# MengLcool/RichSem

Measured on AMD Instinct MI355X. Metric: training images/sec, RichSem R50 4-scale 1333x800 (MSDeformAttn hot path: 12 fwd + 12 bwd calls per step), higher is better.
Workload: dtype f32; 1 GPU; configs[1]: R50 4-scale 800x1344 (S=22323), bs=2/GPU, M=8 D=32 L=P=4; per step 6x E(Lq=22323) + 6x Dd(Lq=1092), forward and backward, 12 distinct per-layer tensor sets; loc-init; loc=init, images_per_gpu=2, parallelism=dp1 (replicas, no collective)

## Files before the change

richsem_amd/csrc/msda_direct.h:

```cpp
#pragma once

#include "msda_common.h"
#include "msda_prep.h"

namespace msda {

struct DirectGeom {
    int N, S, M, D, L, Lq, P;
    int G, logG, nchunks;
    int qtile, ntiles;
    int pbatch;
    unsigned gv_skip;
};

constexpr int kDirectThreads = 256;
constexpr int kDirectWaves = kDirectThreads / kWave;
constexpr int kMinGroup = 8;

template <typename T>
inline size_t direct_lds_bytes(const DirectGeom &g)
{
    const int ipw = kWave / g.G;
    return sizeof(LevelGeom) * g.L + sizeof(PointRec<T>) * kDirectWaves * ipw * (g.pbatch + 1);
}

__device__ __forceinline__ void load_levels(LevelGeom *lv, const int64_t *shapes, const int64_t *lsi, int L)
{
    for (int l = threadIdx.x; l < L; l += blockDim.x) {
        lv[l].H = (int)shapes[2 * l];
        lv[l].W = (int)shapes[2 * l + 1];
        lv[l].start = (int)lsi[l];
        lv[l].pad = 0;
    }
    __syncthreads();
}

template <typename T, int C, int OCC, typename TV = T>
__global__ __launch_bounds__(kDirectThreads, OCC) void fwd_direct_kernel(
    const TV *__restrict__ value, const int64_t *__restrict__ shapes, const int64_t *__restrict__ lsi,
    const T *__restrict__ loc, const T *__restrict__ aw, TV *__restrict__ out, const DirectGeom g)
{
    extern __shared__ __attribute__((aligned(16))) unsigned char smem[];
    LevelGeom *lv = reinterpret_cast<LevelGeom *>(smem);
    PointRec<T> *recs = reinterpret_cast<PointRec<T> *>(smem + sizeof(LevelGeom) * g.L);

    int pair, tile;
    if (!decode_block(blockIdx.x, g.N * g.M, g.ntiles, pair, tile)) return;
    load_levels(lv, shapes, lsi, g.L);

    const int b = pair / g.M, m = pair - b * g.M;
    const int lane = threadIdx.x & (kWave - 1), wave = threadIdx.x / kWave;
    const int ipw = kWave >> g.logG;
    const int j = lane & (g.G - 1);
    const int slot = wave * ipw + (lane >> g.logG);
    const int LP = g.L * g.P;
    const int row_elems = g.M * g.D;
    PointRec<T> *my = recs + slot * (g.pbatch + 1);

    const int q_end = min((tile + 1) * g.qtile, g.Lq);
    for (int q0 = tile * g.qtile; q0 < q_end; q0 += kDirectWaves * ipw) {
        const int q = q0 + slot;
        const bool live = q < q_end;
        const int item = (b * g.Lq + q) * g.M + m;
        for (int ch = 0; ch < g.nchunks; ++ch) {
            const int c0 = (ch * g.G + j) * C;
            const bool has_c = live && c0 < g.D;
            T acc[C];
#pragma unroll
            for (int c = 0; c < C; ++c) acc[c] = (T)0;
            for (int p0 = 0; p0 < LP; p0 += g.pbatch) {
                const int np = min(g.pbatch, LP - p0);
                if (live) {
                    for (int pt = j; pt < np; pt += g.G) {
                        const int gp = p0 + pt, l = gp / g.P;
                        const Pack<T, 2> xy = *reinterpret_cast<const Pack<T, 2> *>(loc + ((int64_t)item * LP + gp) * 2);
                        const T a = aw[(int64_t)item * LP + gp];
                        const LevelGeom G_ = lv[l];
                        PointRec<T> r;
                        T lh, lw;
                        resolve_point<T>(xy.v[0], xy.v[1], G_.H, G_.W,
                                         (b * g.S + G_.start) * row_elems + m * g.D,
                                         row_elems, r.o, lh, lw);
                        const T hh = (T)1 - lh, hw = (T)1 - lw;
                        r.f[0] = hh * hw * a;
                        r.f[1] = hh * lw * a;
                        r.f[2] = lh * hw * a;
                        r.f[3] = lh * lw * a;
                        my[pt] = r;
                    }
                }
                __builtin_amdgcn_wave_barrier();
                if (has_c) {
#pragma unroll(OCC >= 6 ? 2 : 4)
                    for (int pt = 0; pt < np; ++pt) {
                        const PointRec<T> r = my[pt];
                        Pack<T, C> v[4];
#pragma unroll
                        for (int k = 0; k < 4; ++k) {
                            if (r.o[k] >= 0) {
                                const Pack<TV, C> raw = *reinterpret_cast<const Pack<TV, C> *>(value + r.o[k] + c0);
#pragma unroll
                                for (int c = 0; c < C; ++c) v[k].v[c] = to_compute<T, TV>(raw.v[c]);
                            } else {
#pragma unroll
                                for (int c = 0; c < C; ++c) v[k].v[c] = (T)0;
                            }
                        }
#pragma unroll
                        for (int c = 0; c < C; ++c)
                            acc[c] += r.f[0] * v[0].v[c] + r.f[1] * v[1].v[c] + r.f[2] * v[2].v[c] + r.f[3] * v[3].v[c];
                    }
                }
                __builtin_amdgcn_wave_barrier();
            }
            if (has_c) {
                Pack<TV, C> o;
#pragma unroll
                for (int c = 0; c < C; ++c) o.v[c] = to_storage<TV, T>(acc[c]);
                *reinterpret_cast<Pack<TV, C> *>(out + (int64_t)item * g.D + c0) = o;
            }
        }
    }
}

constexpr int kSplitGroups = 4;
constexpr int kSplitMaxPts = 8;
template <typename TV, int PPG>
__global__ __launch_bounds__(kDirectThreads, 4) void fwd_split_kernel(
    const TV *__restrict__ value, const int64_t *__restrict__ shapes, const int64_t *__restrict__ lsi,
    const float *__restrict__ loc, const float *__restrict__ aw, TV *__restrict__ out, const DirectGeom g)
{
    extern __shared__ __attribute__((aligned(16))) unsigned char smem[];
    LevelGeom *lv = reinterpret_cast<LevelGeom *>(smem);
    load_levels(lv, shapes, lsi, g.L);
    const int lane = threadIdx.x & (kWave - 1);
    const int j = lane & 7, pg = (lane >> 3) & (kSplitGroups - 1);
    const long long n_items = (long long)g.N * g.Lq * g.M;
    const long long item_raw = ((long long)blockIdx.x * kDirectThreads + threadIdx.x) >> 5;
    const bool live = item_raw < n_items;
    const long long item = live ? item_raw : n_items - 1;
    const int m = (int)(item % g.M);
    const int b = (int)(item / ((long long)g.Lq * g.M));
    const int LP = g.L * g.P, ppg = PPG ? PPG : LP / kSplitGroups;
    const int row_elems = g.M * g.D, c0 = 4 * j;
    float acc[4] = {0.f, 0.f, 0.f, 0.f};
#pragma unroll
    for (int i = 0; i < (PPG ? PPG : kSplitMaxPts); ++i) {
        if (!PPG && i >= ppg) break;
        const int gp = pg * ppg + i, l = gp / g.P;
        const Pack<float, 2> xy = *reinterpret_cast<const Pack<float, 2> *>(loc + (item * LP + gp) * 2);
        const float a = aw[item * LP + gp];
        const LevelGeom G_ = lv[l];
        int o[4];
        float lh, lw;
        resolve_point<float>(xy.v[0], xy.v[1], G_.H, G_.W, (b * g.S + G_.start) * row_elems + m * g.D, row_elems, o, lh, lw);
        const float hh = 1.f - lh, hw = 1.f - lw;
        const float f[4] = {hh * hw * a, hh * lw * a, lh * hw * a, lh * lw * a};
#pragma unroll
        for (int k = 0; k < 4; ++k) {
            const Pack<TV, 4> raw = *reinterpret_cast<const Pack<TV, 4> *>(value + (o[k] >= 0 ? o[k] : (b * g.S) * row_elems + m * g.D) + c0);
#pragma unroll
            for (int c = 0; c < 4; ++c) acc[c] += f[k] * (o[k] >= 0 ? to_compute<float, TV>(raw.v[c]) : 0.f);
        }
    }
#pragma unroll
    for (int c = 0; c < 4; ++c) {
        acc[c] += dpp_f<0x128>(acc[c]);
        acc[c] += __shfl_xor(acc[c], 16, kWave);
    }
    if (live && pg == 0) {
        Pack<TV, 4> o_;
#pragma unroll
        for (int c = 0; c < 4; ++c) o_.v[c] = to_storage<TV, float>(acc[c]);
        *reinterpret_cast<Pack<TV, 4> *>(out + item * g.D + c0) = o_;
    }
}

template <typename TP>
struct PrepSrc {
    const TP *offsets, *logits;
    long long off_stride, log_stride;
    int ref_dim;
};

template <typename T, int C, int OCC, typename TV, typename TP>
__global__ __launch_bounds__(kDirectThreads, OCC) void fwd_direct_prep_kernel(
    const TV *__restrict__ value, const int64_t *__restrict__ shapes, const int64_t *__restrict__ lsi, const PrepSrc<TP> src,
    const T *__restrict__ ref, T *__restrict__ loc_out, T *__restrict__ aw_out, TV *__restrict__ out, const DirectGeom g)
{
    extern __shared__ __attribute__((aligned(16))) unsigned char smem[];
    LevelGeom *lv = reinterpret_cast<LevelGeom *>(smem);
    PointRec<T> *recs = reinterpret_cast<PointRec<T> *>(smem + sizeof(LevelGeom) * g.L);

    int pair, tile;
    if (!decode_block(blockIdx.x, g.N * g.M, g.ntiles, pair, tile)) return;
    load_levels(lv, shapes, lsi, g.L);

    const int b = pair / g.M, m = pair - b * g.M;
    const int lane = threadIdx.x & (kWave - 1), wave = threadIdx.x / kWave;
    const int ipw = kWave >> g.logG;
    const int j = lane & (g.G - 1);
    const int slot = wave * ipw + (lane >> g.logG);
    const int LP = g.L * g.P;
    const int row_elems = g.M * g.D;
    PointRec<T> *my = recs + slot * (g.pbatch + 1);
    constexpr int kPerLane = kPointBatch / kMinGroup;

    const int q_end = min((tile + 1) * g.qtile, g.Lq);
    for (int q0 = tile * g.qtile; q0 < q_end; q0 += kDirectWaves * ipw) {
        const int q = q0 + slot;
        const bool live = q < q_end;
        const long long nq = (long long)b * g.Lq + (live ? q : q_end - 1);
        const long long item = nq * g.M + m;
        T lg[kPerLane];
        T mx = (T)-3.0e38;
#pragma unroll
        for (int i = 0; i < kPerLane; ++i) {
            const int pt = j + i * g.G;
            lg[i] = pt < LP ? prep_ld<T>(src.logits + nq * src.log_stride + (long long)m * LP + pt) : (T)-3.0e38;
            mx = lg[i] > mx ? lg[i] : mx;
        }
        for (int s_ = 1; s_ < g.G; s_ <<= 1) {
            const T o = __shfl_xor(mx, s_, kWave);
            mx = o > mx ? o : mx;
        }
        T sum = (T)0;
#pragma unroll
        for (int i = 0; i < kPerLane; ++i) {
            lg[i] = j + i * g.G < LP ? exp(lg[i] - mx) : (T)0;
            sum += lg[i];
        }
        for (int s_ = 1; s_ < g.G; s_ <<= 1) sum += __shfl_xor(sum, s_, kWave);
#pragma unroll
        for (int i = 0; i < kPerLane; ++i) {
            const int pt = j + i * g.G;
            if (live && pt < LP) {
                const int l = pt / g.P;
                const T a = lg[i] / sum;
                const TP *o = src.offsets + nq * src.off_stride + ((long long)m * LP + pt) * 2;
                const T ox = prep_ld<T>(o), oy = prep_ld<T>(o + 1);
                const T *r = ref + (nq * g.L + l) * src.ref_dim;
                const LevelGeom G_ = lv[l];
                T lx, ly;
                if (src.ref_dim == 2) {
                    lx = r[0] + ox / (T)G_.W;
                    ly = r[1] + oy / (T)G_.H;
                } else {
                    lx = r[0] + ox / (T)g.P * r[2] * (T)0.5;
                    ly = r[1] + oy / (T)g.P * r[3] * (T)0.5;
                }
                if (loc_out) {
                    Pack<T, 2> xy;
                    xy.v[0] = lx;
                    xy.v[1] = ly;
                    *reinterpret_cast<Pack<T, 2> *>(loc_out + (item * LP + pt) * 2) = xy;
                    aw_out[item * LP + pt] = a;
                }
                PointRec<T> rec;
                T lh, lw;
                resolve_point<T>(lx, ly, G_.H, G_.W, (b * g.S + G_.start) * row_elems + m * g.D, row_elems, rec.o, lh, lw);
                const T hh = (T)1 - lh, hw = (T)1 - lw;
                rec.f[0] = hh * hw * a;
                rec.f[1] = hh * lw * a;
                rec.f[2] = lh * hw * a;
                rec.f[3] = lh * lw * a;
                my[pt] = rec;
            }
        }
        __builtin_amdgcn_wave_barrier();
        for (int ch = 0; ch < g.nchunks; ++ch) {
            const int c0 = (ch * g.G + j) * C;
            if (live && c0 < g.D) {
                T acc[C];
#pragma unroll
                for (int c = 0; c < C; ++c) acc[c] = (T)0;
#pragma unroll(OCC >= 6 ? 2 : 4)
                for (int pt = 0; pt < LP; ++pt) {
                    const PointRec<T> r = my[pt];
                    Pack<T, C> v[4];
#pragma unroll
                    for (int k = 0; k < 4; ++k) {
                        if (r.o[k] >= 0) {
                            const Pack<TV, C> raw = *reinterpret_cast<const Pack<TV, C> *>(value + r.o[k] + c0);
#pragma unroll
                            for (int c = 0; c < C; ++c) v[k].v[c] = to_compute<T, TV>(raw.v[c]);
                        } else {
#pragma unroll
                            for (int c = 0; c < C; ++c) v[k].v[c] = (T)0;
                        }
                    }
#pragma unroll
                    for (int c = 0; c < C; ++c)
                        acc[c] += r.f[0] * v[0].v[c] + r.f[1] * v[1].v[c] + r.f[2] * v[2].v[c] + r.f[3] * v[3].v[c];
                }
                Pack<TV, C> o;
#pragma unroll
                for (int c = 0; c < C; ++c) o.v[c] = to_storage<TV, T>(acc[c]);
                *reinterpret_cast<Pack<TV, C> *>(out + item * g.D + c0) = o;
            }
        }
        __builtin_amdgcn_wave_barrier();
    }
}

template <typename TV, int PPG, int THREADS>
__device__ __forceinline__ void bwd_split_body(unsigned bid, const LevelGeom *lv, const TV *__restrict__ value,
                                               const float *__restrict__ loc, const float *__restrict__ aw, const TV *__restrict__ grad_out,
                                               float *__restrict__ grad_loc, float *__restrict__ grad_aw, const DirectGeom &g)
{
    const int lane = threadIdx.x & (kWave - 1);
    const int j = lane & 7, pg = (lane >> 3) & (kSplitGroups - 1);
    const long long n_items = (long long)g.N * g.Lq * g.M;
    const long long item_raw = ((long long)bid * THREADS + threadIdx.x) >> 5;
    const bool live = item_raw < n_items;
    const long long item = live ? item_raw : n_items - 1;
    const int m = (int)(item % g.M);
    const int b = (int)(item / ((long long)g.Lq * g.M));
    const int LP = g.L * g.P, ppg = PPG ? PPG : LP / kSplitGroups;
    const int row_elems = g.M * g.D, c0 = 4 * j;
    float go[4];
    {
        const Pack<TV, 4> raw = *reinterpret_cast<const Pack<TV, 4> *>(grad_out + item * g.D + c0);
#pragma unroll
        for (int c = 0; c < 4; ++c) go[c] = to_compute<float, TV>(raw.v[c]);
    }
    float r_a[PPG ? PPG : kSplitMaxPts], r_w[PPG ? PPG : kSplitMaxPts], r_h[PPG ? PPG : kSplitMaxPts];
#pragma unroll
    for (int i = 0; i < (PPG ? PPG : kSplitMaxPts); ++i) {
        if (!PPG && i >= ppg) break;
        const int gp = pg * ppg + i, l = gp / g.P;
        const Pack<float, 2> xy = *reinterpret_cast<const Pack<float, 2> *>(loc + (item * LP + gp) * 2);
        const float a = aw[item * LP + gp];
        const LevelGeom G_ = lv[l];
        int o[4];
        float lh, lw;
        resolve_point<float>(xy.v[0], xy.v[1], G_.H, G_.W, (b * g.S + G_.start) * row_elems + m * g.D, row_elems, o, lh, lw);
        const float hh = 1.f - lh, hw = 1.f - lw;
        float v[4][4];
#pragma unroll
        for (int k = 0; k < 4; ++k) {
            const Pack<TV, 4> raw = *reinterpret_cast<const Pack<TV, 4> *>(value + (o[k] >= 0 ? o[k] : (b * g.S) * row_elems + m * g.D) + c0);
#pragma unroll
            for (int c = 0; c < 4; ++c) v[k][c] = o[k] >= 0 ? to_compute<float, TV>(raw.v[c]) : 0.f;
        }
        float s_a = 0.f, s_w = 0.f, s_h = 0.f;
#pragma unroll
        for (int c = 0; c < 4; ++c) {
            const float tgv = go[c] * a;
            s_a += go[c] * (hh * hw * v[0][c] + hh * lw * v[1][c] + lh * hw * v[2][c] + lh * lw * v[3][c]);
            s_w += (hh * (v[1][c] - v[0][c]) + lh * (v[3][c] - v[2][c])) * tgv;
            s_h += (hw * (v[2][c] - v[0][c]) + lw * (v[3][c] - v[1][c])) * tgv;
        }
        r_a[i] = group8_sum(s_a);
        r_w[i] = (float)G_.W * group8_sum(s_w);
        r_h[i] = (float)G_.H * group8_sum(s_h);
        if (!PPG && live && j == 0) {
            grad_aw[item * LP + gp] = r_a[i];
            Pack<float, 2> gl;
            gl.v[0] = r_w[i];
            gl.v[1] = r_h[i];
            *reinterpret_cast<Pack<float, 2> *>(grad_loc + (item * LP + gp) * 2) = gl;
        }
    }
    if (PPG && live && j == 0) {
#pragma unroll
        for (int i = 0; i < PPG; ++i) {
            const int gp = pg * PPG + i;
            grad_aw[item * LP + gp] = r_a[i];
            Pack<float, 2> gl;
            gl.v[0] = r_w[i];
            gl.v[1] = r_h[i];
            *reinterpret_cast<Pack<float, 2> *>(grad_loc + (item * LP + gp) * 2) = gl;
        }
    }
}

template <typename TV, int PPG>
__global__ __launch_bounds__(kDirectThreads, 4) void bwd_split_kernel(
    const TV *__restrict__ value, const int64_t *__restrict__ shapes, const int64_t *__restrict__ lsi,
    const float *__restrict__ loc, const float *__restrict__ aw, const TV *__restrict__ grad_out,
    float *__restrict__ grad_loc, float *__restrict__ grad_aw, const DirectGeom g)
{
    extern __shared__ __attribute__((aligned(16))) unsigned char smem[];
    LevelGeom *lv = reinterpret_cast<LevelGeom *>(smem);
    load_levels(lv, shapes, lsi, g.L);
    bwd_split_body<TV, PPG, kDirectThreads>(blockIdx.x, lv, value, loc, aw, grad_out, grad_loc, grad_aw, g);
}

template <typename T, int C, typename TV = T>
__global__ __launch_bounds__(kDirectThreads) void bwd_direct_kernel(
    const TV *__restrict__ value, const int64_t *__restrict__ shapes, const int64_t *__restrict__ lsi,
    const T *__restrict__ loc, const T *__restrict__ aw, const TV *__restrict__ grad_out,
    T *__restrict__ grad_value, T *__restrict__ grad_loc, T *__restrict__ grad_aw, const DirectGeom g)
{
    extern __shared__ __attribute__((aligned(16))) unsigned char smem[];
    LevelGeom *lv = reinterpret_cast<LevelGeom *>(smem);
    PointRec<T> *recs = reinterpret_cast<PointRec<T> *>(smem + sizeof(LevelGeom) * g.L);

    int pair, tile;
    if (!decode_block(blockIdx.x, g.N * g.M, g.ntiles, pair, tile)) return;
    load_levels(lv, shapes, lsi, g.L);

    const int b = pair / g.M, m = pair - b * g.M;
    const int lane = threadIdx.x & (kWave - 1), wave = threadIdx.x / kWave;
    const int ipw = kWave >> g.logG;
    const int j = lane & (g.G - 1);
    const int slot = wave * ipw + (lane >> g.logG);
    const int LP = g.L * g.P;
    const int row_elems = g.M * g.D;
    PointRec<T> *my = recs + slot * (g.pbatch + 1);

    const int q_end = min((tile + 1) * g.qtile, g.Lq);
    for (int q0 = tile * g.qtile; q0 < q_end; q0 += kDirectWaves * ipw) {
        const int q = q0 + slot;
        const bool live = q < q_end;
        const int item = (b * g.Lq + q) * g.M + m;
        Pack<T, C> g0;
#pragma unroll
        for (int c = 0; c < C; ++c) g0.v[c] = (T)0;
        if (live && j * C < g.D) {
            const Pack<TV, C> raw = *reinterpret_cast<const Pack<TV, C> *>(grad_out + (int64_t)item * g.D + j * C);
#pragma unroll
            for (int c = 0; c < C; ++c) g0.v[c] = to_compute<T, TV>(raw.v[c]);
        }

        for (int p0 = 0; p0 < LP; p0 += g.pbatch) {
            const int np = min(g.pbatch, LP - p0);
            if (live) {
                for (int pt = j; pt < np; pt += g.G) {
                    const int gp = p0 + pt, l = gp / g.P;
                    const Pack<T, 2> xy = *reinterpret_cast<const Pack<T, 2> *>(loc + ((int64_t)item * LP + gp) * 2);
                    const LevelGeom G_ = lv[l];
                    PointRec<T> r;
                    resolve_point<T>(xy.v[0], xy.v[1], G_.H, G_.W, (b * g.S + G_.start) * row_elems + m * g.D,
                                     row_elems, r.o, r.f[0], r.f[1]);
                    r.f[2] = aw[(int64_t)item * LP + gp];
                    r.f[3] = (T)0;
                    my[pt] = r;
                }
            }
            __builtin_amdgcn_wave_barrier();
            for (int pt = 0; pt < np; ++pt) {
                const PointRec<T> r = my[pt];
                const bool add_gv = !((g.gv_skip >> ((p0 + pt) / g.P)) & 1u);
                const T lh = r.f[0], lw = r.f[1], a = r.f[2];
                const T hh = (T)1 - lh, hw = (T)1 - lw;
                const T w[4] = {hh * hw, hh * lw, lh * hw, lh * lw};
                T s_a = (T)0, s_w = (T)0, s_h = (T)0;
                for (int ch = 0; ch < g.nchunks; ++ch) {
                    const int c0 = (ch * g.G + j) * C;
                    if (!(live && c0 < g.D)) continue;
                    Pack<T, C> tg = g0;
                    if (ch > 0) {
                        const Pack<TV, C> raw = *reinterpret_cast<const Pack<TV, C> *>(grad_out + (int64_t)item * g.D + c0);
#pragma unroll
                        for (int c = 0; c < C; ++c) tg.v[c] = to_compute<T, TV>(raw.v[c]);
                    }
                    Pack<T, C> v[4];
#pragma unroll
                    for (int k = 0; k < 4; ++k) {
                        if (r.o[k] >= 0) {
                            const Pack<TV, C> raw = *reinterpret_cast<const Pack<TV, C> *>(value + r.o[k] + c0);
#pragma unroll
                            for (int c = 0; c < C; ++c) v[k].v[c] = to_compute<T, TV>(raw.v[c]);
                        } else {
#pragma unroll
                            for (int c = 0; c < C; ++c) v[k].v[c] = (T)0;
                        }
                    }
#pragma unroll
                    for (int c = 0; c < C; ++c) {
                        const T tgv = tg.v[c] * a;
                        const T v1 = v[0].v[c], v2 = v[1].v[c], v3 = v[2].v[c], v4 = v[3].v[c];
                        s_a += tg.v[c] * (w[0] * v1 + w[1] * v2 + w[2] * v3 + w[3] * v4);
                        s_w += (hh * (v2 - v1) + lh * (v4 - v3)) * tgv;
                        s_h += (hw * (v3 - v1) + lw * (v4 - v2)) * tgv;
#pragma unroll
                        for (int k = 0; k < 4; ++k)
                            if (add_gv && r.o[k] >= 0) atomicAdd(grad_value + r.o[k] + c0 + c, w[k] * tgv);
                    }
                }
                for (int s = 1; s < g.G; s <<= 1) {
                    s_a += shfl_xor_t(s_a, s);
                    s_w += shfl_xor_t(s_w, s);
                    s_h += shfl_xor_t(s_h, s);
                }
                if (live && j == 0) {
                    const int gp = p0 + pt;
                    const LevelGeom G_ = lv[gp / g.P];
                    grad_aw[(int64_t)item * LP + gp] = s_a;
                    Pack<T, 2> gl;
                    gl.v[0] = (T)G_.W * s_w;
                    gl.v[1] = (T)G_.H * s_h;
                    *reinterpret_cast<Pack<T, 2> *>(grad_loc + ((int64_t)item * LP + gp) * 2) = gl;
                }
            }
            __builtin_amdgcn_wave_barrier();
        }
    }
}

}
```

richsem_amd/csrc/msda_levelsum.h:

```cpp
#pragma once

#include <atomic>

#include "msda_common.h"

namespace msda {

constexpr int kLsChan = 4;
constexpr int kLsThreads = 1024;
constexpr int kLsMaxLevels = 32;
constexpr int kLsUnroll = 4;
constexpr int kLsLdsBudget = 150 * 1024;
inline std::atomic<int> &levelsum_lds_kb()
{
    static std::atomic<int> kb{150};
    return kb;
}

struct LevelSumGeom {
    int N, S, M, D, L, Lq, P;
    int nlev, nslices;
    int lev[kLsMaxLevels], H[kLsMaxLevels], W[kLsMaxLevels], start[kLsMaxLevels], r0[kLsMaxLevels], nr[kLsMaxLevels];
};

inline unsigned plan_levelsum(int N, int S, int M, int D, int L, int Lq, int P, const int64_t *shapes,
                              const int64_t *lsi, LevelSumGeom &g, size_t &lds_bytes, int budget_kb = 0)
{
    lds_bytes = 0;
    if (L > 32 || D > 128 || (int64_t)Lq * P > 1048576) { g = LevelSumGeom{}; return 0; }
    const size_t px_bytes = (size_t)kLsChan * sizeof(double);
    const size_t budget = std::min<size_t>(kLsLdsBudget, (size_t)std::max(8, budget_kb ? budget_kb : levelsum_lds_kb().load()) * 1024);
    for (int all = 1; all >= 0; --all) {
        g = LevelSumGeom{};
        g.N = N; g.S = S; g.M = M; g.D = D; g.L = L; g.Lq = Lq; g.P = P;
        g.nslices = (D + kLsChan - 1) / kLsChan;
        lds_bytes = 0;
        unsigned mask = 0;
        bool ok = true;
        for (int l = 0; l < L && ok; ++l) {
            const int H = (int)shapes[2 * l], W = (int)shapes[2 * l + 1];
            const int64_t px = (int64_t)H * W;
            const bool whole = px * px_bytes <= budget;
            if (!all && (!whole || (int64_t)Lq * P < 2 * px)) continue;
            const int rows_max = (int)(budget / (px_bytes * W));
            if (rows_max < 1) { ok = false; break; }
            const int bands = whole ? 1 : (H + rows_max - 1) / rows_max;
            const int rows = (H + bands - 1) / bands;
            if (bands > 16 || g.nlev + bands > kLsMaxLevels) { ok = false; break; }
            for (int r0 = 0; r0 < H; r0 += rows) {
                const int e = g.nlev++;
                g.lev[e] = l; g.H[e] = H; g.W[e] = W; g.start[e] = (int)lsi[l];
                g.r0[e] = r0;
                g.nr[e] = H - r0 < rows ? H - r0 : rows;
                const size_t bytes = (size_t)g.nr[e] * W * px_bytes;
                lds_bytes = bytes > lds_bytes ? bytes : lds_bytes;
            }
            mask |= 1u << l;
        }
        if (all && (!ok || mask != (L >= 32 ? ~0u : (1u << L) - 1))) continue;
        return mask;
    }
    g = LevelSumGeom{};
    return 0;
}

inline int levelsum_grid(const LevelSumGeom &g)
{
    return kXcds * ((g.N * g.M + kXcds - 1) / kXcds) * g.nlev * g.nslices;
}

template <bool P4, typename TV, int THREADS>
__device__ __forceinline__ void levelsum_body(int bid, double *win, const float *loc, const float *aw, const TV *grad_out,
                                              TV *grad_value, const LevelSumGeom g)
{
    int pair, t;
    if (!decode_block(bid, g.N * g.M, g.nlev * g.nslices, pair, t)) return;
    const int li = g.nlev - 1 - t / g.nslices, slice = t - (t / g.nslices) * g.nslices;
    const int b = pair / g.M, m = pair - b * g.M;
    const int l = g.lev[li], H = g.H[li], W = g.W[li], r0 = g.r0[li], nr = g.nr[li];
    const int npx = nr * W;
    const int tid = threadIdx.x;
    const int j = tid & (kLsChan - 1), grp = tid / kLsChan;
    constexpr int kGroups = THREADS / kLsChan;
    const int ch = slice * kLsChan + j;
    const bool has_ch = ch < g.D;

    for (int e = tid; e < npx * kLsChan; e += THREADS) win[e] = 0.0;
    __syncthreads();

    const int LP = g.L * g.P;
    for (int q = grp; q < g.Lq; q += kGroups) {
        const unsigned item = (unsigned)((b * g.Lq + q) * g.M + m);
        const unsigned pt0 = item * (unsigned)LP + (unsigned)(l * g.P);
        const float go = has_ch ? ld1(grad_out + item * (unsigned)g.D + ch) : 0.f;
        if (P4) {
            static_assert(kLsChan == 4, "one quad per query");
            const float2 xy = *reinterpret_cast<const float2 *>(loc + 2u * (pt0 + (unsigned)j));
            const float a = aw[pt0 + (unsigned)j];
            const float h_im = xy.y * (float)H - 0.5f, w_im = xy.x * (float)W - 0.5f;
            const float hf = floorf(h_im), wf = floorf(w_im);
            const int h_low = (int)hf, w_low = (int)wf;
            const float lh = h_im - hf, lw = w_im - wf, hh = 1.f - lh, hw = 1.f - lw;
            const bool top = h_low >= r0 && h_low < r0 + nr, bot = h_low + 1 >= r0 && h_low + 1 < r0 + nr;
            const bool alive = h_im > -1.f && w_im > -1.f && h_im < (float)H && w_im < (float)W && (top || bot);
            const bool lef = w_low >= 0, rig = w_low + 1 <= W - 1;
            const int rt = (top ? h_low : h_low + 1) - r0, rb = (bot ? h_low + 1 : h_low) - r0;
            const int cl = lef ? w_low : w_low + 1, cr = rig ? w_low + 1 : w_low;
            const int my_o[4] = {(rt * W + cl) * kLsChan, (rt * W + cr) * kLsChan, (rb * W + cl) * kLsChan, (rb * W + cr) * kLsChan};
            const float my_w[4] = {top && lef ? hh * hw : 0.f, top && rig ? hh * lw : 0.f, bot && lef ? lh * hw : 0.f, bot && rig ? lh * lw : 0.f};
#define LS_BCAST_I(V, K) __builtin_amdgcn_update_dpp(0, (V), (K) * 0x55, 0xF, 0xF, true)
#define LS_BCAST_F(V, K) __int_as_float(__builtin_amdgcn_update_dpp(0, __float_as_int(V), (K) * 0x55, 0xF, 0xF, true))
#define LS_POINT(K)                                                                                     \
    if (LS_BCAST_I((int)alive, K)) {                                                                    \
        const float ga_ = go * LS_BCAST_F(a, K);  \
        atomicAdd(win + LS_BCAST_I(my_o[0], K) + j, (double)(LS_BCAST_F(my_w[0], K) * ga_));            \
        atomicAdd(win + LS_BCAST_I(my_o[1], K) + j, (double)(LS_BCAST_F(my_w[1], K) * ga_));            \
        atomicAdd(win + LS_BCAST_I(my_o[2], K) + j, (double)(LS_BCAST_F(my_w[2], K) * ga_));            \
        atomicAdd(win + LS_BCAST_I(my_o[3], K) + j, (double)(LS_BCAST_F(my_w[3], K) * ga_));            \
    }
            LS_POINT(0)
            LS_POINT(1)
            LS_POINT(2)
            LS_POINT(3)
#undef LS_POINT
#undef LS_BCAST_I
#undef LS_BCAST_F
            continue;
        }
        for (int p0 = 0; p0 < g.P; p0 += kLsUnroll) {
            float x[kLsUnroll], y[kLsUnroll], ga[kLsUnroll];
            {
#pragma unroll
                for (int u = 0; u < kLsUnroll; ++u) {
                    const bool live = p0 + u < g.P;
                    const unsigned pt = pt0 + (unsigned)(live ? p0 + u : 0);
                    const float2 xy = *reinterpret_cast<const float2 *>(loc + 2u * pt);
                    const float a = aw[pt];
                    x[u] = live ? xy.x : -4.f;
                    y[u] = xy.y;
                    ga[u] = go * a;
                }
            }
#pragma unroll
            for (int u = 0; u < kLsUnroll; ++u) {
                const float h_im = y[u] * (float)H - 0.5f, w_im = x[u] * (float)W - 0.5f;
                if (!(h_im > -1.f && w_im > -1.f && h_im < (float)H && w_im < (float)W)) continue;
                const float hf = floorf(h_im), wf = floorf(w_im);
                const int h_low = (int)hf, w_low = (int)wf;
                const float lh = h_im - hf, lw = w_im - wf, hh = 1.f - lh, hw = 1.f - lw;
                const bool top = h_low >= r0 && h_low < r0 + nr, bot = h_low + 1 >= r0 && h_low + 1 < r0 + nr;
                if (!(top || bot)) continue;
                const bool lef = w_low >= 0, rig = w_low + 1 <= W - 1;
                const int rt = (top ? h_low : h_low + 1) - r0, rb = (bot ? h_low + 1 : h_low) - r0;
                const int cl = lef ? w_low : w_low + 1, cr = rig ? w_low + 1 : w_low;
                double *pt_ = win + (rt * W) * kLsChan + j, *pb_ = win + (rb * W) * kLsChan + j;
                atomicAdd(pt_ + cl * kLsChan, (double)(top && lef ? hh * hw * ga[u] : 0.f));
                atomicAdd(pt_ + cr * kLsChan, (double)(top && rig ? hh * lw * ga[u] : 0.f));
                atomicAdd(pb_ + cl * kLsChan, (double)(bot && lef ? lh * hw * ga[u] : 0.f));
                atomicAdd(pb_ + cr * kLsChan, (double)(bot && rig ? lh * lw * ga[u] : 0.f));
            }
        }
    }
    __syncthreads();

    TV *dst = grad_value + ((int64_t)(b * g.S + g.start[li] + r0 * W) * g.M + m) * g.D + ch;
    if (has_ch)
        for (int px = grp; px < npx; px += kGroups) dst[(int64_t)px * g.M * g.D] = to_storage<TV, float>((float)win[px * kLsChan + j]);
}

template <bool P4, typename TV = float>
__global__ __launch_bounds__(kLsThreads) void bwd_levelsum_kernel(const float *__restrict__ loc,
                                                                  const float *__restrict__ aw,
                                                                  const TV *__restrict__ grad_out,
                                                                  TV *__restrict__ grad_value, const LevelSumGeom g)
{
    extern __shared__ __attribute__((aligned(16))) unsigned char smem[];
    levelsum_body<P4, TV, kLsThreads>(blockIdx.x, reinterpret_cast<double *>(smem), loc, aw, grad_out, grad_value, g);
}

}
```

Before: 754.2 img/s.

## Software-pipeline gathers in split backward and levelsum kernels, bf16 raw loads

The split backward kernel now issues all corner gathers for a point group before computing, or prefetches the next point's loc/aw in the dynamic-PPG path. Empty asm constraints pin the loaded registers so the compiler cannot sink the loads back next to their uses. The levelsum P4 path prefetches the next query's grad_out, loc and aw while it processes the current one, and the window zeroing is moved after the first issue. bf16 values are loaded as raw dwords and unpacked inline; the cost is higher register pressure and a changed FMA order in the backward sums.

```diff
diff --git a/richsem_amd/csrc/msda_direct.h b/richsem_amd/csrc/msda_direct.h
--- a/richsem_amd/csrc/msda_direct.h
+++ b/richsem_amd/csrc/msda_direct.h
@@ -123,6 +123,21 @@
     }
 }
 
+template <typename TV>
+struct RawRow;
+template <>
+struct RawRow<float> {
+    typedef Pack<float, 4> reg;
+    static __device__ __forceinline__ float get(const reg &r, int c) { return r.v[c]; }
+    static __device__ __forceinline__ void pin(reg &r) { asm volatile("" : "+v"(r.v[0]), "+v"(r.v[1]), "+v"(r.v[2]), "+v"(r.v[3])); }
+};
+template <>
+struct RawRow<bf16_t> {
+    typedef unsigned reg __attribute__((ext_vector_type(2)));
+    static __device__ __forceinline__ float get(const reg &r, int c) { return __uint_as_float(c & 1 ? r[c >> 1] & 0xffff0000u : r[c >> 1] << 16); }
+    static __device__ __forceinline__ void pin(reg &r) { asm volatile("" : "+v"(r)); }
+};
+
 constexpr int kSplitGroups = 4;
 constexpr int kSplitMaxPts = 8;
 template <typename TV, int PPG>
@@ -158,9 +173,9 @@
         const float f[4] = {hh * hw * a, hh * lw * a, lh * hw * a, lh * lw * a};
 #pragma unroll
         for (int k = 0; k < 4; ++k) {
-            const Pack<TV, 4> raw = *reinterpret_cast<const Pack<TV, 4> *>(value + (o[k] >= 0 ? o[k] : (b * g.S) * row_elems + m * g.D) + c0);
-#pragma unroll
-            for (int c = 0; c < 4; ++c) acc[c] += f[k] * (o[k] >= 0 ? to_compute<float, TV>(raw.v[c]) : 0.f);
+            const typename RawRow<TV>::reg raw = *reinterpret_cast<const typename RawRow<TV>::reg *>(value + (o[k] >= 0 ? o[k] : (b * g.S) * row_elems + m * g.D) + c0);
+#pragma unroll
+            for (int c = 0; c < 4; ++c) acc[c] += f[k] * (o[k] >= 0 ? RawRow<TV>::get(raw, c) : 0.f);
         }
     }
 #pragma unroll
@@ -303,6 +318,50 @@
     }
 }
 
+template <typename TV>
+struct SplitCorners {
+    typename RawRow<TV>::reg raw[4];
+    unsigned inside;
+    float lh, lw;
+    __device__ __forceinline__ void gather(const TV *__restrict__ value, const Pack<float, 2> &xy, const LevelGeom &G_, int base_row, int row_elems,
+                                           int own_row, int c0)
+    {
+        int o[4];
+        resolve_point<float>(xy.v[0], xy.v[1], G_.H, G_.W, base_row, row_elems, o, lh, lw);
+        inside = 0;
+#pragma unroll
+        for (int k = 0; k < 4; ++k) {
+            raw[k] = *reinterpret_cast<const typename RawRow<TV>::reg *>(value + (o[k] >= 0 ? o[k] : own_row) + c0);
+            inside |= (o[k] >= 0 ? 1u : 0u) << k;
+        }
+    }
+    __device__ __forceinline__ void pin()
+    {
+#pragma unroll
+        for (int k = 0; k < 4; ++k) RawRow<TV>::pin(raw[k]);
+    }
+    __device__ __forceinline__ void sums(const float (&go)[4], float a, float &s_a, float &s_w, float &s_h) const
+    {
+#pragma clang fp contract(off)
+        const float hh = 1.f - lh, hw = 1.f - lw;
+        float v[4][4];
+#pragma unroll
+        for (int k = 0; k < 4; ++k)
+#pragma unroll
+            for (int c = 0; c < 4; ++c) v[k][c] = inside >> k & 1u ? RawRow<TV>::get(raw[k], c) : 0.f;
+        const float w0 = hh * hw, w1 = hh * lw, w2 = lh * hw, w3 = lh * lw;
+        s_a = s_w = s_h = 0.f;
+#pragma unroll
+        for (int c = 0; c < 4; ++c) {
+            const float tgv = go[c] * a;
+            const float t = __builtin_fmaf(w3, v[3][c], __builtin_fmaf(w2, v[2][c], __builtin_fmaf(w0, v[0][c], w1 * v[1][c])));
+            s_a = __builtin_fmaf(go[c], t, s_a);
+            s_w = __builtin_fmaf(__builtin_fmaf(hh, v[1][c] - v[0][c], lh * (v[3][c] - v[2][c])), tgv, s_w);
+            s_h = __builtin_fmaf(__builtin_fmaf(hw, v[2][c] - v[0][c], lw * (v[3][c] - v[1][c])), tgv, s_h);
+        }
+    }
+};
+
 template <typename TV, int PPG, int THREADS>
 __device__ __forceinline__ void bwd_split_body(unsigned bid, const LevelGeom *lv, const TV *__restrict__ value,
                                                const float *__restrict__ loc, const float *__restrict__ aw, const TV *__restrict__ grad_out,
@@ -324,53 +383,73 @@
 #pragma unroll
         for (int c = 0; c < 4; ++c) go[c] = to_compute<float, TV>(raw.v[c]);
     }
-    float r_a[PPG ? PPG : kSplitMaxPts], r_w[PPG ? PPG : kSplitMaxPts], r_h[PPG ? PPG : kSplitMaxPts];
-#pragma unroll
-    for (int i = 0; i < (PPG ? PPG : kSplitMaxPts); ++i) {
-        if (!PPG && i >= ppg) break;
-        const int gp = pg * ppg + i, l = gp / g.P;
-        const Pack<float, 2> xy = *reinterpret_cast<const Pack<float, 2> *>(loc + (item * LP + gp) * 2);
-        const float a = aw[item * LP + gp];
-        const LevelGeom G_ = lv[l];
-        int o[4];
-        float lh, lw;
-        resolve_point<float>(xy.v[0], xy.v[1], G_.H, G_.W, (b * g.S + G_.start) * row_elems + m * g.D, row_elems, o, lh, lw);
-        const float hh = 1.f - lh, hw = 1.f - lw;
-        float v[4][4];
-#pragma unroll
-        for (int k = 0; k < 4; ++k) {
-            const Pack<TV, 4> raw = *reinterpret_cast<const Pack<TV, 4> *>(value + (o[k] >= 0 ? o[k] : (b * g.S) * row_elems + m * g.D) + c0);
-#pragma unroll
-            for (int c = 0; c < 4; ++c) v[k][c] = o[k] >= 0 ? to_compute<float, TV>(raw.v[c]) : 0.f;
-        }
-        float s_a = 0.f, s_w = 0.f, s_h = 0.f;
-#pragma unroll
-        for (int c = 0; c < 4; ++c) {
-            const float tgv = go[c] * a;
-            s_a += go[c] * (hh * hw * v[0][c] + hh * lw * v[1][c] + lh * hw * v[2][c] + lh * lw * v[3][c]);
-            s_w += (hh * (v[1][c] - v[0][c]) + lh * (v[3][c] - v[2][c])) * tgv;
-            s_h += (hw * (v[2][c] - v[0][c]) + lw * (v[3][c] - v[1][c])) * tgv;
-        }
-        r_a[i] = group8_sum(s_a);
-        r_w[i] = (float)G_.W * group8_sum(s_w);
-        r_h[i] = (float)G_.H * group8_sum(s_h);
-        if (!PPG && live && j == 0) {
-            grad_aw[item * LP + gp] = r_a[i];
-            Pack<float, 2> gl;
-            gl.v[0] = r_w[i];
-            gl.v[1] = r_h[i];
-            *reinterpret_cast<Pack<float, 2> *>(grad_loc + (item * LP + gp) * 2) = gl;
-        }
-    }
-    if (PPG && live && j == 0) {
+    const int own_row = (b * g.S) * row_elems + m * g.D;
+    if constexpr (PPG != 0) {
+        Pack<float, 2> xy[PPG];
+        float a[PPG];
 #pragma unroll
         for (int i = 0; i < PPG; ++i) {
             const int gp = pg * PPG + i;
-            grad_aw[item * LP + gp] = r_a[i];
-            Pack<float, 2> gl;
-            gl.v[0] = r_w[i];
-            gl.v[1] = r_h[i];
-            *reinterpret_cast<Pack<float, 2> *>(grad_loc + (item * LP + gp) * 2) = gl;
+            xy[i] = *reinterpret_cast<const Pack<float, 2> *>(loc + (item * LP + gp) * 2);
+            a[i] = aw[item * LP + gp];
+        }
+        SplitCorners<TV> cn[PPG];
+#pragma unroll
+        for (int i = 0; i < PPG; ++i) {
+            const LevelGeom G_ = lv[(pg * PPG + i) / g.P];
+            cn[i].gather(value, xy[i], G_, (b * g.S + G_.start) * row_elems + m * g.D, row_elems, own_row, c0);
+        }
+#pragma unroll
+        for (int i = 0; i < PPG; ++i) cn[i].pin();
+        float r_a[PPG], r_w[PPG], r_h[PPG];
+#pragma unroll
+        for (int i = 0; i < PPG; ++i) {
+            const LevelGeom G_ = lv[(pg * PPG + i) / g.P];
+            float s_a, s_w, s_h;
+            cn[i].sums(go, a[i], s_a, s_w, s_h);
+            r_a[i] = group8_sum(s_a);
+            r_w[i] = (float)G_.W * group8_sum(s_w);
+            r_h[i] = (float)G_.H * group8_sum(s_h);
+        }
+        if (live && j == 0) {
+#pragma unroll
+            for (int i = 0; i < PPG; ++i) {
+                const int gp = pg * PPG + i;
+                grad_aw[item * LP + gp] = r_a[i];
+                Pack<float, 2> gl;
+                gl.v[0] = r_w[i];
+                gl.v[1] = r_h[i];
+                *reinterpret_cast<Pack<float, 2> *>(grad_loc + (item * LP + gp) * 2) = gl;
+            }
+        }
+    } else {
+        Pack<float, 2> xy = *reinterpret_cast<const Pack<float, 2> *>(loc + (item * LP + pg * ppg) * 2);
+        float a = aw[item * LP + pg * ppg];
+#pragma unroll
+        for (int i = 0; i < kSplitMaxPts; ++i) {
+            if (i >= ppg) break;
+            const int gp = pg * ppg + i;
+            const LevelGeom G_ = lv[gp / g.P];
+            SplitCorners<TV> cn;
+            cn.gather(value, xy, G_, (b * g.S + G_.start) * row_elems + m * g.D, row_elems, own_row, c0);
+            const float a_now = a;
+            const int gn = pg * ppg + min(i + 1, ppg - 1);
+            xy = *reinterpret_cast<const Pack<float, 2> *>(loc + (item * LP + gn) * 2);
+            a = aw[item * LP + gn];
+            cn.pin();
+            float s_a, s_w, s_h;
+            cn.sums(go, a_now, s_a, s_w, s_h);
+            s_a = group8_sum(s_a);
+            s_w = (float)G_.W * group8_sum(s_w);
+            s_h = (float)G_.H * group8_sum(s_h);
+            asm volatile("" : "+v"(xy.v[0]), "+v"(xy.v[1]), "+v"(a));
+            if (live && j == 0) {
+                grad_aw[item * LP + gp] = s_a;
+                Pack<float, 2> gl;
+                gl.v[0] = s_w;
+                gl.v[1] = s_h;
+                *reinterpret_cast<Pack<float, 2> *>(grad_loc + (item * LP + gp) * 2) = gl;
+            }
         }
     }
 }
diff --git a/richsem_amd/csrc/msda_levelsum.h b/richsem_amd/csrc/msda_levelsum.h
--- a/richsem_amd/csrc/msda_levelsum.h
+++ b/richsem_amd/csrc/msda_levelsum.h
@@ -85,24 +85,34 @@
     const int ch = slice * kLsChan + j;
     const bool has_ch = ch < g.D;
 
-    for (int e = tid; e < npx * kLsChan; e += THREADS) win[e] = 0.0;
-    __syncthreads();
-
     const int LP = g.L * g.P;
-    for (int q = grp; q < g.Lq; q += kGroups) {
-        const unsigned item = (unsigned)((b * g.Lq + q) * g.M + m);
-        const unsigned pt0 = item * (unsigned)LP + (unsigned)(l * g.P);
-        const float go = has_ch ? ld1(grad_out + item * (unsigned)g.D + ch) : 0.f;
-        if (P4) {
-            static_assert(kLsChan == 4, "one quad per query");
-            const float2 xy = *reinterpret_cast<const float2 *>(loc + 2u * (pt0 + (unsigned)j));
-            const float a = aw[pt0 + (unsigned)j];
+    if constexpr (P4) {
+        static_assert(kLsChan == 4, "one quad per query");
+        const int ch_ld = has_ch ? ch : g.D - 1;
+        float go, a, go_n, a_n;
+        float2 xy, xy_n;
+        auto issue = [&](int q, float &go_, float2 &xy_, float &a_) {
+            const unsigned item = (unsigned)((b * g.Lq + min(q, g.Lq - 1)) * g.M + m);
+            const unsigned pt = item * (unsigned)LP + (unsigned)(l * g.P) + (unsigned)j;
+            go_ = ld1(grad_out + item * (unsigned)g.D + ch_ld);
+            xy_ = *reinterpret_cast<const float2 *>(loc + 2u * pt);
+            a_ = aw[pt];
+        };
+        int q = grp;
+        issue(q, go, xy, a);
+        for (int e = tid; e < npx * kLsChan; e += THREADS) win[e] = 0.0;
+        __syncthreads();
+        for (;;) {
+            const int qn = q + kGroups;
+            issue(qn, go_n, xy_n, a_n);
+            asm volatile("" : "+v"(go), "+v"(xy.x), "+v"(xy.y), "+v"(a));
+            const float go_ = has_ch ? go : 0.f;
             const float h_im = xy.y * (float)H - 0.5f, w_im = xy.x * (float)W - 0.5f;
             const float hf = floorf(h_im), wf = floorf(w_im);
             const int h_low = (int)hf, w_low = (int)wf;
             const float lh = h_im - hf, lw = w_im - wf, hh = 1.f - lh, hw = 1.f - lw;
             const bool top = h_low >= r0 && h_low < r0 + nr, bot = h_low + 1 >= r0 && h_low + 1 < r0 + nr;
-            const bool alive = h_im > -1.f && w_im > -1.f && h_im < (float)H && w_im < (float)W && (top || bot);
+            const bool alive = q < g.Lq && h_im > -1.f && w_im > -1.f && h_im < (float)H && w_im < (float)W && (top || bot);
             const bool lef = w_low >= 0, rig = w_low + 1 <= W - 1;
             const int rt = (top ? h_low : h_low + 1) - r0, rb = (bot ? h_low + 1 : h_low) - r0;
             const int cl = lef ? w_low : w_low + 1, cr = rig ? w_low + 1 : w_low;
@@ -112,7 +122,7 @@
 #define LS_BCAST_F(V, K) __int_as_float(__builtin_amdgcn_update_dpp(0, __float_as_int(V), (K) * 0x55, 0xF, 0xF, true))
 #define LS_POINT(K)                                                                                     \
     if (LS_BCAST_I((int)alive, K)) {                                                                    \
-        const float ga_ = go * LS_BCAST_F(a, K);  \
+        const float ga_ = go_ * LS_BCAST_F(a, K);  \
         atomicAdd(win + LS_BCAST_I(my_o[0], K) + j, (double)(LS_BCAST_F(my_w[0], K) * ga_));            \
         atomicAdd(win + LS_BCAST_I(my_o[1], K) + j, (double)(LS_BCAST_F(my_w[1], K) * ga_));            \
         atomicAdd(win + LS_BCAST_I(my_o[2], K) + j, (double)(LS_BCAST_F(my_w[2], K) * ga_));            \
@@ -125,39 +135,52 @@
 #undef LS_POINT
 #undef LS_BCAST_I
 #undef LS_BCAST_F
-            continue;
+            q = qn;
+            if (q >= g.Lq) break;
+            go = go_n;
+            xy = xy_n;
+            a = a_n;
         }
-        for (int p0 = 0; p0 < g.P; p0 += kLsUnroll) {
-            float x[kLsUnroll], y[kLsUnroll], ga[kLsUnroll];
-            {
+    } else {
+        for (int e = tid; e < npx * kLsChan; e += THREADS) win[e] = 0.0;
+        __syncthreads();
+
+        for (int q = grp; q < g.Lq; q += kGroups) {
+            const unsigned item = (unsigned)((b * g.Lq + q) * g.M + m);
+            const unsigned pt0 = item * (unsigned)LP + (unsigned)(l * g.P);
+            const float go = has_ch ? ld1(grad_out + item * (unsigned)g.D + ch) : 0.f;
+            for (int p0 = 0; p0 < g.P; p0 += kLsUnroll) {
+                float x[kLsUnroll], y[kLsUnroll], ga[kLsUnroll];
+                {
+#pragma unroll
+                    for (int u = 0; u < kLsUnroll; ++u) {
+                        const bool live = p0 + u < g.P;
+                        const unsigned pt = pt0 + (unsigned)(live ? p0 + u : 0);
+                        const float2 xy = *reinterpret_cast<const float2 *>(loc + 2u * pt);
+                        const float a = aw[pt];
+                        x[u] = live ? xy.x : -4.f;
+                        y[u] = xy.y;
+                        ga[u] = go * a;
+                    }
+                }
 #pragma unroll
                 for (int u = 0; u < kLsUnroll; ++u) {
-                    const bool live = p0 + u < g.P;
-                    const unsigned pt = pt0 + (unsigned)(live ? p0 + u : 0);
-                    const float2 xy = *reinterpret_cast<const float2 *>(loc + 2u * pt);
-                    const float a = aw[pt];
-                    x[u] = live ? xy.x : -4.f;
-                    y[u] = xy.y;
-                    ga[u] = go * a;
+                    const float h_im = y[u] * (float)H - 0.5f, w_im = x[u] * (float)W - 0.5f;
+                    if (!(h_im > -1.f && w_im > -1.f && h_im < (float)H && w_im < (float)W)) continue;
+                    const float hf = floorf(h_im), wf = floorf(w_im);
+                    const int h_low = (int)hf, w_low = (int)wf;
+                    const float lh = h_im - hf, lw = w_im - wf, hh = 1.f - lh, hw = 1.f - lw;
+                    const bool top = h_low >= r0 && h_low < r0 + nr, bot = h_low + 1 >= r0 && h_low + 1 < r0 + nr;
+                    if (!(top || bot)) continue;
+                    const bool lef = w_low >= 0, rig = w_low + 1 <= W - 1;
+                    const int rt = (top ? h_low : h_low + 1) - r0, rb = (bot ? h_low + 1 : h_low) - r0;
+                    const int cl = lef ? w_low : w_low + 1, cr = rig ? w_low + 1 : w_low;
+                    double *pt_ = win + (rt * W) * kLsChan + j, *pb_ = win + (rb * W) * kLsChan + j;
+                    atomicAdd(pt_ + cl * kLsChan, (double)(top && lef ? hh * hw * ga[u] : 0.f));
+                    atomicAdd(pt_ + cr * kLsChan, (double)(top && rig ? hh * lw * ga[u] : 0.f));
+                    atomicAdd(pb_ + cl * kLsChan, (double)(bot && lef ? lh * hw * ga[u] : 0.f));
+                    atomicAdd(pb_ + cr * kLsChan, (double)(bot && rig ? lh * lw * ga[u] : 0.f));
                 }
-            }
-#pragma unroll
-            for (int u = 0; u < kLsUnroll; ++u) {
-                const float h_im = y[u] * (float)H - 0.5f, w_im = x[u] * (float)W - 0.5f;
-                if (!(h_im > -1.f && w_im > -1.f && h_im < (float)H && w_im < (float)W)) continue;
-                const float hf = floorf(h_im), wf = floorf(w_im);
-                const int h_low = (int)hf, w_low = (int)wf;
-                const float lh = h_im - hf, lw = w_im - wf, hh = 1.f - lh, hw = 1.f - lw;
-                const bool top = h_low >= r0 && h_low < r0 + nr, bot = h_low + 1 >= r0 && h_low + 1 < r0 + nr;
-                if (!(top || bot)) continue;
-                const bool lef = w_low >= 0, rig = w_low + 1 <= W - 1;
-                const int rt = (top ? h_low : h_low + 1) - r0, rb = (bot ? h_low + 1 : h_low) - r0;
-                const int cl = lef ? w_low : w_low + 1, cr = rig ? w_low + 1 : w_low;
-                double *pt_ = win + (rt * W) * kLsChan + j, *pb_ = win + (rb * W) * kLsChan + j;
-                atomicAdd(pt_ + cl * kLsChan, (double)(top && lef ? hh * hw * ga[u] : 0.f));
-                atomicAdd(pt_ + cr * kLsChan, (double)(top && rig ? hh * lw * ga[u] : 0.f));
-                atomicAdd(pb_ + cl * kLsChan, (double)(bot && lef ? lh * hw * ga[u] : 0.f));
-                atomicAdd(pb_ + cr * kLsChan, (double)(bot && rig ? lh * lw * ga[u] : 0.f));
             }
         }
     }
```

Result: no change. 762.5 img/s (median of 6 runs) (+1.1%).
